# skit-ai/N-Best-ASR-Transformer

Hardware: AMD Instinct MI355X
Metric: utterances/sec fine-tune (bert-base, seq128, n_best=5) (higher is better)
Workload: dtype bf16

## Files before the change

### n-best-asr-transformer_amd/csrc/attention.hip

```cpp
#include "common.h"

namespace {

__device__ __forceinline__ int crow(int reg, int hh) { return (reg & 3) + 8 * (reg >> 2) + 4 * hh; }
__device__ __forceinline__ int gsw(int row) { return ((row >> 2) & 3) | (((row >> 1) & 1) << 2); }

__global__ __launch_bounds__(128) void attn_fwd_f32_kernel(const float* __restrict__ qkv, const uint8_t* __restrict__ mask,
                                                           float* __restrict__ ctx, float* __restrict__ lse, int S, int heads,
                                                           int H, float scale, DropCfg drop) {
  const int bh = blockIdx.x, b = bh / heads, h = bh - b * heads;
  const int i = blockIdx.y * blockDim.x + threadIdx.x;
  if (i >= S) return;
  const int64_t ld = 3 * (int64_t)H;
  const float* base = qkv + (int64_t)b * S * ld;
  const float* qp = base + i * ld + h * 64;
  float q[64];
#pragma unroll
  for (int d = 0; d < 64; ++d) q[d] = qp[d];
  float mx = -INFINITY, l = 0.f;
  for (int j = 0; j < S; ++j) {
    if (!mask[b * S + j]) continue;
    const float* kp = base + j * ld + H + h * 64;
    float s = 0.f;
#pragma unroll
// ... 232 lines not shown
  for (int qb = wave; qb < (kOne ? wave + 1 : NKB); qb += 4) {
    const int q0 = 32 * qb, qrow = q0 + (lane & 31);
    const bool active = qb < NKB;
    if (!kOne) load_q(qb, qf);
    f32x16 sc[NKB];
    if (active) {
#pragma unroll
    for (int kb = 0; kb < NKB; ++kb) {
      f32x16 a;
#pragma unroll
      for (int r = 0; r < 16; ++r) a[r] = 0.f;
#pragma unroll
      for (int ks = 0; ks < 4; ++ks) a = __builtin_amdgcn_mfma_f32_32x32x16_bf16(row_frag(Kt, 32 * kb, ks, lane), qf[ks], a, 0, 0, 0);
      sc[kb] = a;
    }
    }
    if (kOne) __syncthreads();
    if (!active) continue;
    float mx = -INFINITY;
#pragma unroll
    for (int kb = 0; kb < NKB; ++kb)
#pragma unroll
      for (int r4 = 0; r4 < 4; ++r4) {
        const f32x4 ma = *(const f32x4*)(madd + 32 * kb + 8 * r4 + 4 * hh);
#pragma unroll
        for (int e = 0; e < 4; ++e) {
          const float v = sc[kb][4 * r4 + e] * sl2 + ma[e];
          sc[kb][4 * r4 + e] = v;
          mx = fmaxf(mx, v);
        }
      }
    mx = fmaxf(mx, __shfl_xor(mx, 32, 64));
    const float mxs = (mx == -INFINITY) ? 0.f : mx;
    float sum = 0.f;
#pragma unroll
    for (int kb = 0; kb < NKB; ++kb)
#pragma unroll
      for (int r = 0; r < 16; ++r) {
        const float pv = __builtin_amdgcn_exp2f(sc[kb][r] - mxs);
        sc[kb][r] = pv;
        sum += pv;
      }
    sum += __shfl_xor(sum, 32, 64);
    const float inv = 1.0f / sum;
    if (hh == 0 && qrow < S) lse[(int64_t)bh * S + qrow] = mxs * 0.6931471805599453f + __logf(sum);
    bf16x8 pa[NKB][2];
    if (DROP && drop.thr16 && (S & 1) == 0) {
      const uint32_t rowbase = (uint32_t)((bh * S + qrow) * S);
      const uint32_t hb = ((rowbase >> 1) + 2u * (uint32_t)hh) * 0x9E3779B9U + drop.key;
      const float ids = inv * drop.scale;
#pragma unroll
      for (int kb = 0; kb < NKB; ++kb) {
        uint32_t kw = 0;
#pragma unroll
        for (int r = 0; r < 16; r += 2) {
          const uint32_t hsh = nb_hash32(hb + (uint32_t)((32 * kb + crow(r, 0)) >> 1) * 0x9E3779B9U);
          const bool k0 = (hsh & 0xFFFFu) >= drop.thr16, k1 = (hsh >> 16) >= drop.thr16;
          const float p0 = k0 ? sc[kb][r] * ids : 0.f;
          const float p1 = k1 ? sc[kb][r + 1] * ids : 0.f;
          kw |= (k0 ? (1u << crow(r, 0)) : 0u) | (k1 ? (2u << crow(r, 0)) : 0u);
          pa[kb][r >> 3][r & 7] = (bf16)p0;
          pa[kb][r >> 3][(r & 7) + 1] = (bf16)p1;
        }
        if (keep_out) {
          kw <<= 4 * hh;
          kw |= (uint32_t)__shfl_xor((int)kw, 32, 64);
          if (hh == 0 && qrow < Sp) keep_out[((int64_t)bh * NKB + kb) * Sp + qrow] = kw;
        }
      }
    } else {
#pragma unroll
      for (int kb = 0; kb < NKB; ++kb) {
        uint32_t kw = 0;
#pragma unroll
        for (int r = 0; r < 16; ++r) {
          float pv = sc[kb][r] * inv;
          if (DROP && drop.thr16) {
            const int key = 32 * kb + crow(r, hh);
            const bool kp = nb_keep(drop, (uint32_t)((bh * S + qrow) * S + key));
            pv = kp ? pv * drop.scale : 0.f;
            kw |= kp ? (1u << crow(r, hh)) : 0u;
          }
          pa[kb][r >> 3][r & 7] = (bf16)pv;
        }
        if (DROP && keep_out && drop.thr16) {
          kw |= (uint32_t)__shfl_xor((int)kw, 32, 64);
          if (hh == 0 && qrow < Sp) keep_out[((int64_t)bh * NKB + kb) * Sp + qrow] = kw;
        }
      }
    }
    f32x16 o0, o1;
#pragma unroll
    for (int r = 0; r < 16; ++r) o0[r] = o1[r] = 0.f;
#pragma unroll
    for (int kb = 0; kb < NKB; ++kb)
#pragma unroll
      for (int s = 0; s < 2; ++s) {
        o0 = __builtin_amdgcn_mfma_f32_32x32x16_bf16(pa[kb][s], tr_frag<true>(Vt, 32 * kb + 16 * s, 0, lane), o0, 0, 0, 0);
        o1 = __builtin_amdgcn_mfma_f32_32x32x16_bf16(pa[kb][s], tr_frag<true>(Vt, 32 * kb + 16 * s, 32, lane), o1, 0, 0, 0);
      }
    store_tile(Ost + wave * 4096, 0, o0, o1, lane, ctx + ((int64_t)b * S + q0) * H + h * 64, H, S - q0,
               ctx8 ? ctx8 + ((int64_t)b * S + q0) * H + h * 64 : nullptr, s8, amax8, a_new != nullptr);
  }
  if (a_new) {
    amax8 = wave_max(amax8);
    if (lane == 0) amax_update(a_new, amax8);
  }
}

template <int NKB, bool KB>
__global__ __launch_bounds__((NKB <= 4 ? 4 : 8) * 64, 2) void attn_bwd2_bf16_kernel(
    const bf16* __restrict__ qkv, const uint8_t* __restrict__ mask, const bf16* __restrict__ ctx, const bf16* __restrict__ dctx,
    const float* __restrict__ lse, bf16* __restrict__ dqkv, float* __restrict__ colpart, int S, int heads, int H, float scale,
    DropCfg drop, Fp8Grad f8, const uint32_t* __restrict__ keep) {
  extern __shared__ __attribute__((aligned(16))) char lds[];
  constexpr int Sp = NKB * 32;
  constexpr int NW = (NKB <= 4) ? 4 : 8, NT = NW * 64;
  char* Qt = lds;
  char* Kt = Qt + Sp * 128;
  char* dOt = Kt + Sp * 128;
  char* dST = dOt + Sp * 128;
  float* lse_s = (float*)(dST + Sp * 128);
  float* del_s = lse_s + Sp;
  uint32_t* kw_s = (uint32_t*)(del_s + Sp);
  const int tid = threadIdx.x, lane = tid & 63, wave = tid >> 6, hh = lane >> 5;
  const int bh = blockIdx.x, b = bh / heads, h = bh - b * heads;
  const int ld = 3 * H;
  const bf16* base = qkv + (int64_t)b * S * ld;
  const bf16* dobase = dctx + (int64_t)b * S * H;
  const bf16* obase = ctx + (int64_t)b * S * H;
  const __amdgpu_buffer_rsrc_t rs = __builtin_amdgcn_make_buffer_rsrc((void*)base, 0, (uint32_t)(S * ld * 2), 0x00020000);
  const __amdgpu_buffer_rsrc_t rsd = __builtin_amdgcn_make_buffer_rsrc((void*)dobase, 0, (uint32_t)(S * H * 2), 0x00020000);
  stage_rows(rs, Qt, Sp, h * 64, ld, tid, NT);
  stage_rows(rs, Kt, Sp, H + h * 64, ld, tid, NT);
  stage_rows(rsd, dOt, Sp, h * 64, H, tid, NT);
  for (int k = tid; k < Sp; k += NT) lse_s[k] = (k < S) ? lse[(int64_t)bh * S + k] * 1.4426950408889634f : INFINITY;
  if (KB) {
    for (int i = tid; i < NKB * Sp; i += NT) kw_s[i] = keep[(int64_t)bh * NKB * Sp + i];
  }
  {
    const int r = tid >> 1, half = tid & 1;
    float sdel = 0.f;
    if (r < S) {
      const bf16* dp = dobase + (int64_t)r * H + h * 64 + 32 * half;
      const bf16* op = obase + (int64_t)r * H + h * 64 + 32 * half;
#pragma unroll
      for (int c = 0; c < 4; ++c) {
        float a[8], o[8];
        Vec8<bf16>::load(dp + 8 * c, a);
        Vec8<bf16>::load(op + 8 * c, o);
#pragma unroll
        for (int j = 0; j < 8; ++j) sdel = fmaf(a[j], o[j], sdel);
      }
    }
    sdel += __shfl_xor(sdel, 1, 64);
    if (half == 0 && r < Sp) del_s[r] = sdel;
  }
  const int key = 32 * wave + (lane & 31);
  const bool kvalid = (wave < NKB) && key < S;
  const float mk = (kvalid && mask[b * S + key]) ? 0.f : -INFINITY;
  const uint32_t lanebit = 1u << (lane & 31);
  const float sl2 = scale * 1.4426950408889634f;
  bf16x8 kf[4], vf[4];
#pragma unroll
  for (int ks = 0; ks < 4; ++ks) {
    const i32x4 raw = kvalid ? *(const i32x4*)(base + (int64_t)key * ld + 2 * H + h * 64 + 16 * ks + 8 * hh) : i32x4{0, 0, 0, 0};
    vf[ks] = __builtin_bit_cast(bf16x8, raw);
  }
  asm volatile("s_waitcnt vmcnt(0)" ::: "memory");
  __syncthreads();
  if (wave < NKB) {
#pragma unroll
    for (int ks = 0; ks < 4; ++ks) kf[ks] = row_frag(Kt, 32 * wave, ks, lane);
  }
  f32x16 dk0, dk1, dv0, dv1, dq0, dq1;
#pragma unroll
  for (int r = 0; r < 16; ++r) dk0[r] = dk1[r] = dv0[r] = dv1[r] = dq0[r] = dq1[r] = 0.f;
  char* dsrow = dST + key * 128;
  const int dsg = gsw(key);

#pragma unroll 1
  for (int qb = 0; qb < NKB; ++qb) {
    const int half = qb & 1;
    if (wave < NKB) {
      f32x16 sa, da;
#pragma unroll
      for (int r = 0; r < 16; ++r) sa[r] = da[r] = 0.f;
#pragma unroll
      for (int ks = 0; ks < 4; ++ks) {
        sa = __builtin_amdgcn_mfma_f32_32x32x16_bf16(row_frag(Qt, 32 * qb, ks, lane), kf[ks], sa, 0, 0, 0);
        da = __builtin_amdgcn_mfma_f32_32x32x16_bf16(row_frag(dOt, 32 * qb, ks, lane), vf[ks], da, 0, 0, 0);
      }
#pragma unroll
      for (int r4 = 0; r4 < 4; ++r4) {
        const int qoff = 32 * qb + 8 * r4 + 4 * hh;
        const f32x4 l4 = *(const f32x4*)(lse_s + qoff);
        const f32x4 d4 = *(const f32x4*)(del_s + qoff);
        i32x4 k4 = {0, 0, 0, 0};
        if (KB) k4 = *(const i32x4*)(kw_s + wave * Sp + qoff);
        bf16x4 pk;
#pragma unroll
        for (int e = 0; e < 4; ++e) {
          const int r = 4 * r4 + e;
          const float pv = __builtin_amdgcn_exp2f(fmaf(sa[r], sl2, mk - l4[e]));
          float pt = pv, dp = da[r];
          if (KB) {
            const float kf_ = ((uint32_t)k4[e] & lanebit) ? drop.scale : 0.f;
            pt = pv * kf_;
            dp = dp * kf_;
          } else if (drop.thr16) {
            const bool keep_ = nb_keep(drop, (uint32_t)((bh * S + qoff + e) * S + key));
            pt = keep_ ? pv * drop.scale : 0.f;
            dp = keep_ ? dp * drop.scale : 0.f;
          }
          const float ds = pv * (dp - d4[e]) * scale;
          sa[r] = pt;
          da[r] = ds;
          pk[e] = (bf16)ds;
        }
        const int col = 32 * half + 8 * r4 + 4 * hh;
        *(bf16x4*)(dsrow + (((col >> 3) ^ dsg) << 4) + ((col & 4) ? 8 : 0)) = pk;
      }
#pragma unroll
      for (int s2 = 0; s2 < 2; ++s2) {
        const bf16x8 pa = acc_to_frag(sa, s2), dsa = acc_to_frag(da, s2);
        dv0 = __builtin_amdgcn_mfma_f32_32x32x16_bf16(pa, tr_frag<true>(dOt, 32 * qb + 16 * s2, 0, lane), dv0, 0, 0, 0);
        dv1 = __builtin_amdgcn_mfma_f32_32x32x16_bf16(pa, tr_frag<true>(dOt, 32 * qb + 16 * s2, 32, lane), dv1, 0, 0, 0);
        dk0 = __builtin_amdgcn_mfma_f32_32x32x16_bf16(dsa, tr_frag<true>(Qt, 32 * qb + 16 * s2, 0, lane), dk0, 0, 0, 0);
        dk1 = __builtin_amdgcn_mfma_f32_32x32x16_bf16(dsa, tr_frag<true>(Qt, 32 * qb + 16 * s2, 32, lane), dk1, 0, 0, 0);
      }
    }
    __syncthreads();
    if (wave == (qb % NW)) {
#pragma unroll
      for (int ks = 0; ks < 2 * NKB; ++ks) {
        const bf16x8 dsf = tr_frag<false>(dST, 16 * ks, 32 * half, lane);
        dq0 = __builtin_amdgcn_mfma_f32_32x32x16_bf16(dsf, tr_frag<false>(Kt, 16 * ks, 0, lane), dq0, 0, 0, 0);
        dq1 = __builtin_amdgcn_mfma_f32_32x32x16_bf16(dsf, tr_frag<false>(Kt, 16 * ks, 32, lane), dq1, 0, 0, 0);
      }
    }
  }
  __syncthreads();
  if (colpart) {
    float* cs = (float*)dST;
    const f32x16* tiles[6] = {&dq0, &dq1, &dk0, &dk1, &dv0, &dv1};
#pragma unroll
    for (int t6 = 0; t6 < 6; ++t6) {
      float x = 0.f;
      if (wave < NKB) {
#pragma unroll
        for (int r = 0; r < 16; ++r) x += (*tiles[t6])[r];
      }
      x += __shfl_xor(x, 32, 64);
      if (lane < 32) cs[(wave * 3 + (t6 >> 1)) * 64 + (t6 & 1) * 32 + lane] = x;
    }
    __syncthreads();
    if (tid < 192) {
      const int which = tid >> 6, dcol = tid & 63;
      float x = 0.f;
#pragma unroll
      for (int w2 = 0; w2 < NW; ++w2) x += cs[(w2 * 3 + which) * 64 + dcol];
      colpart[(int64_t)b * 3 * H + which * H + h * 64 + dcol] = x;
    }
  }
  if (wave < NKB) {
    const int r0 = 32 * wave;
    const int64_t goff = ((int64_t)b * S + r0) * ld + h * 64;
    bf16* g = dqkv ? dqkv + goff : nullptr;
    uint8_t* g8 = f8.out8 ? f8.out8 + goff : nullptr;
    const float s8 = fp8_grad_scale(f8.amax_prev);
    float amax8 = 0.f;
    const bool am = f8.amax_new != nullptr;
    store_tile(Qt, r0, dq0, dq1, lane, g, ld, S - r0, g8, s8, amax8, am);
    store_tile(Kt, r0, dk0, dk1, lane, g ? g + H : nullptr, ld, S - r0, g8 ? g8 + H : nullptr, s8, amax8, am);
    store_tile(dOt, r0, dv0, dv1, lane, g ? g + 2 * H : nullptr, ld, S - r0, g8 ? g8 + 2 * H : nullptr, s8, amax8, am);
    if (f8.amax_new) {
      amax8 = wave_max(amax8);
      if (lane == 0) amax_update(f8.amax_new, amax8);
    }
  }
}


__device__ __forceinline__ bf16x8 row_frag16(const char* tile, int row0, int ks, int lane) {
  const int row = row0 + (lane & 15);
  const int c = 4 * ks + (lane >> 4);
  return *(const bf16x8*)(tile + row * 128 + ((c ^ gsw(row)) << 4));
}
template <bool PERMUTED>
__device__ __forceinline__ bf16x8 tr_frag16(const char* tile, int kbase, int col0, int lane) {
  const int g = lane >> 4, i = lane & 15, qq = i >> 2, pq = i & 3;
  const int col = col0 + 4 * pq;
  const int r1 = kbase + (PERMUTED ? 4 * g : 8 * g) + qq;
  const int r2 = r1 + (PERMUTED ? 16 : 4);
  const char* a1 = tile + r1 * 128 + (((col >> 3) ^ gsw(r1)) << 4) + ((col & 4) ? 8 : 0);
  const char* a2 = tile + r2 * 128 + (((col >> 3) ^ gsw(r2)) << 4) + ((col & 4) ? 8 : 0);
  const bf16x4 v1 = __builtin_amdgcn_ds_read_tr16_b64_v4bf16((bf16x4 __attribute__((address_space(3)))*)a1);
  const bf16x4 v2 = __builtin_amdgcn_ds_read_tr16_b64_v4bf16((bf16x4 __attribute__((address_space(3)))*)a2);
  bf16x8 o;
  o[0] = v1[0]; o[1] = v1[1]; o[2] = v1[2]; o[3] = v1[3]; o[4] = v2[0]; o[5] = v2[1]; o[6] = v2[2]; o[7] = v2[3];
  return o;
}

template <int NKB, bool KB>
__global__ __launch_bounds__(NKB * 128, 4) void attn_bwd3_bf16_kernel(
    const bf16* __restrict__ qkv, const uint8_t* __restrict__ mask, const bf16* __restrict__ ctx, const bf16* __restrict__ dctx,
    const float* __restrict__ lse, bf16* __restrict__ dqkv, float* __restrict__ colpart, int S, int heads, int H, float scale,
    DropCfg drop, Fp8Grad f8, const uint32_t* __restrict__ keep) {
  extern __shared__ __attribute__((aligned(16))) char lds[];
  static_assert(NKB == 4 || NKB == 8, "attn_bwd3: 8 or 16 waves of 16 keys");
  constexpr int Sp = NKB * 32, NW = 2 * NKB, NT = NW * 64;
  char* Qt = lds;
  char* Kt = Qt + Sp * 128;
  char* dOt = Kt + Sp * 128;
  char* dST = dOt + Sp * 128;
  float* lse_s = (float*)(dST + Sp * 128);
  float* del_s = lse_s + Sp;
  uint32_t* kw_s = (uint32_t*)(del_s + Sp);
  const int tid = threadIdx.x, lane = tid & 63, wave = tid >> 6, g = lane >> 4, c16 = lane & 15;
  const int bh = blockIdx.x, b = bh / heads, h = bh - b * heads;
  const int ld = 3 * H;
  const bf16* base = qkv + (int64_t)b * S * ld;
  const bf16* dobase = dctx + (int64_t)b * S * H;
  const bf16* obase = ctx + (int64_t)b * S * H;
  const __amdgpu_buffer_rsrc_t rs = __builtin_amdgcn_make_buffer_rsrc((void*)base, 0, (uint32_t)(S * ld * 2), 0x00020000);
  const __amdgpu_buffer_rsrc_t rsd = __builtin_amdgcn_make_buffer_rsrc((void*)dobase, 0, (uint32_t)(S * H * 2), 0x00020000);
  stage_rows(rs, Qt, Sp, h * 64, ld, tid, NT);
  stage_rows(rs, Kt, Sp, H + h * 64, ld, tid, NT);
  stage_rows(rsd, dOt, Sp, h * 64, H, tid, NT);
  for (int k = tid; k < Sp; k += NT) lse_s[k] = (k < S) ? lse[(int64_t)bh * S + k] * 1.4426950408889634f : INFINITY;
  if (KB) {
    for (int i = tid; i < NKB * Sp; i += NT) kw_s[i] = keep[(int64_t)bh * NKB * Sp + i];
  }
  {
    const int r = tid >> 2, quarter = tid & 3;
    float sdel = 0.f;
    if (r < S) {
      const bf16* dp = dobase + (int64_t)r * H + h * 64 + 16 * quarter;
      const bf16* op = obase + (int64_t)r * H + h * 64 + 16 * quarter;
#pragma unroll
      for (int c = 0; c < 2; ++c) {
        float a[8], o[8];
        Vec8<bf16>::load(dp + 8 * c, a);
        Vec8<bf16>::load(op + 8 * c, o);
#pragma unroll
        for (int j = 0; j < 8; ++j) sdel = fmaf(a[j], o[j], sdel);
      }
    }
    sdel += __shfl_xor(sdel, 1, 64);
    sdel += __shfl_xor(sdel, 2, 64);
    if (quarter == 0 && r < Sp) del_s[r] = sdel;
  }
  const int key = 16 * wave + c16;
  const bool kvalid = key < S;
  const float mk = (kvalid && mask[b * S + key]) ? 0.f : -INFINITY;
  const uint32_t lanebit = 1u << (key & 31);
  const float sl2 = scale * 1.4426950408889634f;
  bf16x8 kf[2], vf[2];
#pragma unroll
  for (int ks = 0; ks < 2; ++ks) {
    const i32x4 raw = kvalid ? *(const i32x4*)(base + (int64_t)key * ld + 2 * H + h * 64 + 32 * ks + 8 * g) : i32x4{0, 0, 0, 0};
    vf[ks] = __builtin_bit_cast(bf16x8, raw);
  }
  asm volatile("s_waitcnt vmcnt(0)" ::: "memory");
  __syncthreads();
#pragma unroll
  for (int ks = 0; ks < 2; ++ks) kf[ks] = row_frag16(Kt, 16 * wave, ks, lane);
  f32x4 dk[4], dv[4], dq[4];
#pragma unroll
  for (int t = 0; t < 4; ++t) { dk[t] = f32x4{0, 0, 0, 0}; dv[t] = f32x4{0, 0, 0, 0}; }
#pragma unroll
  for (int t = 0; t < 4; ++t) dq[t] = f32x4{0, 0, 0, 0};
  char* dsrow = dST + key * 128;
  const int dsg = gsw(key);
  const int qt_mine = (wave & 7) >> 2, dt_mine = wave & 3;
  const int khalf = wave >> 3;

#pragma unroll
  for (int qb = 0; qb < NKB; ++qb) {
    const int half = qb & 1;
    f32x4 sa[2], da[2];
#pragma unroll
    for (int qt = 0; qt < 2; ++qt) {
      sa[qt] = f32x4{0, 0, 0, 0}; da[qt] = f32x4{0, 0, 0, 0};
#pragma unroll
      for (int ks = 0; ks < 2; ++ks) {
        sa[qt] = __builtin_amdgcn_mfma_f32_16x16x32_bf16(row_frag16(Qt, 32 * qb + 16 * qt, ks, lane), kf[ks], sa[qt], 0, 0, 0);
        da[qt] = __builtin_amdgcn_mfma_f32_16x16x32_bf16(row_frag16(dOt, 32 * qb + 16 * qt, ks, lane), vf[ks], da[qt], 0, 0, 0);
      }
    }
    bf16x8 pa, dsa;
#pragma unroll
    for (int qt = 0; qt < 2; ++qt) {
      const int qoff = 32 * qb + 16 * qt + 4 * g;
      const f32x4 l4 = *(const f32x4*)(lse_s + qoff);
      const f32x4 d4 = *(const f32x4*)(del_s + qoff);
      i32x4 k4 = {0, 0, 0, 0};
      if (KB) k4 = *(const i32x4*)(kw_s + (wave >> 1) * Sp + qoff);
      bf16x4 pk;
#pragma unroll
      for (int e = 0; e < 4; ++e) {
        const float pv = __builtin_amdgcn_exp2f(fmaf(sa[qt][e], sl2, mk - l4[e]));
        float pt = pv, dp = da[qt][e];
        if (KB) {
          const float kf_ = ((uint32_t)k4[e] & lanebit) ? drop.scale : 0.f;
          pt = pv * kf_;
          dp = dp * kf_;
        } else if (drop.thr16) {
          const bool keep_ = nb_keep(drop, (uint32_t)((bh * S + qoff + e) * S + key));
          pt = keep_ ? pv * drop.scale : 0.f;
          dp = keep_ ? dp * drop.scale : 0.f;
        }
        const float ds = pv * (dp - d4[e]) * scale;
        pa[4 * qt + e] = (bf16)pt;
        dsa[4 * qt + e] = (bf16)ds;
        pk[e] = (bf16)ds;
      }
      const int col = 32 * half + 16 * qt + 4 * g;
      *(bf16x4*)(dsrow + (((col >> 3) ^ dsg) << 4) + ((col & 4) ? 8 : 0)) = pk;
    }
#pragma unroll
    for (int dt = 0; dt < 4; ++dt) {
      dv[dt] = __builtin_amdgcn_mfma_f32_16x16x32_bf16(pa, tr_frag16<true>(dOt, 32 * qb, 16 * dt, lane), dv[dt], 0, 0, 0);
      dk[dt] = __builtin_amdgcn_mfma_f32_16x16x32_bf16(dsa, tr_frag16<true>(Qt, 32 * qb, 16 * dt, lane), dk[dt], 0, 0, 0);
    }
    __syncthreads();
    if (NKB == 4 || (qb & 1) == khalf) {
      const int slot = (NKB == 4) ? qb : (qb >> 1);
#pragma unroll
      for (int ks = 0; ks < NKB; ++ks)
        dq[slot] = __builtin_amdgcn_mfma_f32_16x16x32_bf16(tr_frag16<false>(dST, 32 * ks, 32 * half + 16 * qt_mine, lane),
                                                           tr_frag16<false>(Kt, 32 * ks, 16 * dt_mine, lane), dq[slot], 0, 0, 0);
    }
  }
  __syncthreads();
  if (colpart) {
    float* cs = (float*)dST;
    float* csq = cs + NW * 2 * 64;
#pragma unroll
    for (int dt = 0; dt < 4; ++dt) {
      float xk = (dk[dt][0] + dk[dt][1]) + (dk[dt][2] + dk[dt][3]);
      float xv = (dv[dt][0] + dv[dt][1]) + (dv[dt][2] + dv[dt][3]);
      xk += __shfl_xor(xk, 16, 64); xk += __shfl_xor(xk, 32, 64);
      xv += __shfl_xor(xv, 16, 64); xv += __shfl_xor(xv, 32, 64);
      if (g == 0) { cs[(wave * 2 + 0) * 64 + 16 * dt + c16] = xk; cs[(wave * 2 + 1) * 64 + 16 * dt + c16] = xv; }
    }
    float xq = 0.f;
#pragma unroll
    for (int t = 0; t < 4; ++t) xq += (dq[t][0] + dq[t][1]) + (dq[t][2] + dq[t][3]);
    xq += __shfl_xor(xq, 16, 64); xq += __shfl_xor(xq, 32, 64);
    if (g == 0) csq[wave * 16 + c16] = xq;
    __syncthreads();
    if (tid < 192) {
      const int which = tid >> 6, dcol = tid & 63;
      float x = 0.f;
      if (which == 0) {
#pragma unroll
        for (int w2 = 0; w2 < NW / 4; ++w2) x += csq[((dcol >> 4) + 4 * w2) * 16 + (dcol & 15)];
      }
      else {
#pragma unroll
        for (int w2 = 0; w2 < NW; ++w2) x += cs[(w2 * 2 + (which - 1)) * 64 + dcol];
      }
      colpart[(int64_t)b * 3 * H + which * H + h * 64 + dcol] = x;
    }
    __syncthreads();
  }
#pragma unroll
  for (int dt = 0; dt < 4; ++dt)
#pragma unroll
    for (int e = 0; e < 4; ++e) {
      const int row = 16 * wave + 4 * g + e;
      *(bf16*)(Kt + row * 128 + (16 * dt + c16) * 2) = (bf16)dk[dt][e];
      *(bf16*)(dOt + row * 128 + (16 * dt + c16) * 2) = (bf16)dv[dt][e];
    }
#pragma unroll
  for (int t = 0; t < 4; ++t) {
    const int qb = (NKB == 4) ? t : 2 * t + khalf;
#pragma unroll
    for (int e = 0; e < 4; ++e)
      *(bf16*)(Qt + (32 * qb + 16 * qt_mine + 4 * g + e) * 128 + (16 * dt_mine + c16) * 2) = (bf16)dq[t][e];
  }
  __syncthreads();
  {
    const int64_t goff = (int64_t)b * S * ld + h * 64;
    bf16* gq = dqkv ? dqkv + goff : nullptr;
    uint8_t* g8 = f8.out8 ? f8.out8 + goff : nullptr;
    const float s8 = fp8_grad_scale(f8.amax_prev);
    const bool am = f8.amax_new != nullptr;
    float amax8 = 0.f;
    const char* imgs[3] = {Qt, Kt, dOt};
#pragma unroll
    for (int t = 0; t < 3; ++t) {
#pragma unroll
      for (int it = 0; it < (Sp * 8) / NT; ++it) {
        const int p = it * NT + tid, row = p >> 3, ch = p & 7;
        if (row < S) {
          const i32x4 v = *(const i32x4*)(imgs[t] + row * 128 + ch * 16);
          if (gq) *(i32x4*)(gq + (int64_t)row * ld + t * H + ch * 8) = v;
          if (g8 || am) {
            const bf16x8 bb = __builtin_bit_cast(bf16x8, v);
            float f[8];
#pragma unroll
            for (int e = 0; e < 8; ++e) f[e] = (float)bb[e];
            if (am) {
#pragma unroll
              for (int e = 0; e < 8; ++e) amax8 = fmaxf(amax8, fabsf(f[e]));
            }
            if (g8) {
#pragma unroll
              for (int e = 0; e < 8; ++e) f[e] *= s8;
              *(i32x2*)(g8 + (int64_t)row * ld + t * H + ch * 8) = i32x2{(int)fp8_pack4(f), (int)fp8_pack4(f + 4)};
            }
          }
        }
      }
    }
    if (am) {
      amax8 = wave_max(amax8);
      if (lane == 0) amax_update(f8.amax_new, amax8);
    }
  }
}


__device__ __forceinline__ void stage_rows_off(__amdgpu_buffer_rsrc_t rs, char* tile, int nrows, int row_off, int col_off, int ld,
                                               int t, int nt) {
  const int chunks = nrows * 8;
  for (int p = t; p < chunks; p += nt) {
    const int row = p >> 3, slot = p & 7;
    const int c = slot ^ gsw(row);
    const uint32_t voff = (uint32_t)(((row_off + row) * ld + col_off + c * 8) * 2);
    __builtin_amdgcn_raw_ptr_buffer_load_lds(rs, LDS_PTR(tile + (p & ~63) * 16), 16, voff, 0, 0, 0);
  }
}

__global__ __launch_bounds__(256) void attn_fwd_long_bf16_kernel(const bf16* __restrict__ qkv, const uint8_t* __restrict__ mask,
                                                                 bf16* __restrict__ ctx, float* __restrict__ lse, int S, int nkb,
                                                                 int heads, int H, float scale, DropCfg drop, uint8_t* __restrict__ ctx8,
                                                                 const uint32_t* __restrict__ a_prev, uint32_t* __restrict__ a_new) {
  const float s8 = fp8_act_scale(a_prev);
  float amax8 = 0.f;
  extern __shared__ __attribute__((aligned(16))) char lds[];
  const int Sp = nkb * 32;
  char* Kt = lds;
  char* Vt = lds + Sp * 128;
  float* madd = (float*)(lds + 2 * Sp * 128);
  char* Ost = lds + 2 * Sp * 128 + Sp * 4;
  const int tid = threadIdx.x, lane = tid & 63, wave = tid >> 6, hh = lane >> 5;
  const int bh = blockIdx.x, b = bh / heads, h = bh - b * heads;
  const int ld = 3 * H;
  const bf16* base = qkv + (int64_t)b * S * ld;
  const __amdgpu_buffer_rsrc_t rs = __builtin_amdgcn_make_buffer_rsrc((void*)base, 0, (uint32_t)(S * ld * 2), 0x00020000);
  stage_rows(rs, Kt, Sp, H + h * 64, ld, tid);
  stage_rows(rs, Vt, Sp, 2 * H + h * 64, ld, tid);
  for (int k = tid; k < Sp; k += 256) madd[k] = (k < S && mask[b * S + k]) ? 0.f : -INFINITY;
  asm volatile("s_waitcnt vmcnt(0)" ::: "memory");
  __syncthreads();

  for (int qb = wave; qb < nkb; qb += 4) {
    const int q0 = 32 * qb, qrow = q0 + (lane & 31);
    bf16x8 qf[4];
#pragma unroll
    for (int ks = 0; ks < 4; ++ks) {
      const i32x4 raw = (qrow < S) ? *(const i32x4*)(base + (int64_t)qrow * ld + h * 64 + 16 * ks + 8 * hh) : i32x4{0, 0, 0, 0};
      qf[ks] = __builtin_bit_cast(bf16x8, raw);
    }
    float m = -INFINITY, l = 0.f;
#pragma unroll 1
    for (int kb = 0; kb < nkb; ++kb) {
      f32x16 a;
#pragma unroll
      for (int r = 0; r < 16; ++r) a[r] = 0.f;
#pragma unroll
      for (int ks = 0; ks < 4; ++ks) a = __builtin_amdgcn_mfma_f32_32x32x16_bf16(row_frag(Kt, 32 * kb, ks, lane), qf[ks], a, 0, 0, 0);
      float bm = -INFINITY;
#pragma unroll
      for (int r4 = 0; r4 < 4; ++r4) {
        const f32x4 ma = *(const f32x4*)(madd + 32 * kb + 8 * r4 + 4 * hh);
#pragma unroll
        for (int e = 0; e < 4; ++e) {
          const float v = a[4 * r4 + e] * scale + ma[e];
          a[4 * r4 + e] = v;
          bm = fmaxf(bm, v);
        }
      }
      const float mn = fmaxf(m, bm);
      if (mn > -INFINITY) {
        float add = 0.f;
#pragma unroll
        for (int r = 0; r < 16; ++r) add += __expf(a[r] - mn);
        l = ((m > -INFINITY) ? l * __expf(m - mn) : 0.f) + add;
      }
      m = mn;
    }
    const float mo = __shfl_xor(m, 32, 64), lo = __shfl_xor(l, 32, 64);
    const float mx = fmaxf(m, mo);
    const float mxs = (mx == -INFINITY) ? 0.f : mx;
    const float sum = ((m > -INFINITY) ? l * __expf(m - mxs) : 0.f) + ((mo > -INFINITY) ? lo * __expf(mo - mxs) : 0.f);
    const float inv = 1.0f / sum;
    if (hh == 0 && qrow < S) lse[(int64_t)bh * S + qrow] = mxs + __logf(sum);
    f32x16 o0, o1;
#pragma unroll
    for (int r = 0; r < 16; ++r) o0[r] = o1[r] = 0.f;
    const uint32_t rowbase = (uint32_t)((bh * S + qrow) * S);
    const bool pair_hash = drop.thr16 && (S & 1) == 0;
#pragma unroll 1
    for (int kb = 0; kb < nkb; ++kb) {
      f32x16 a;
#pragma unroll
      for (int r = 0; r < 16; ++r) a[r] = 0.f;
#pragma unroll
      for (int ks = 0; ks < 4; ++ks) a = __builtin_amdgcn_mfma_f32_32x32x16_bf16(row_frag(Kt, 32 * kb, ks, lane), qf[ks], a, 0, 0, 0);
#pragma unroll
      for (int r4 = 0; r4 < 4; ++r4) {
        const f32x4 ma = *(const f32x4*)(madd + 32 * kb + 8 * r4 + 4 * hh);
#pragma unroll
        for (int e = 0; e < 4; ++e) a[4 * r4 + e] = __expf(a[4 * r4 + e] * scale + ma[e] - mxs) * inv;
      }
      if (pair_hash) {
#pragma unroll
        for (int r = 0; r < 16; r += 2) {
          const uint32_t idx = rowbase + (uint32_t)(32 * kb + crow(r, hh));
          const uint32_t hsh = nb_hash32((idx >> 1) * 0x9E3779B9U + drop.key);
          a[r] = ((hsh & 0xFFFFu) >= drop.thr16) ? a[r] * drop.scale : 0.f;
          a[r + 1] = ((hsh >> 16) >= drop.thr16) ? a[r + 1] * drop.scale : 0.f;
        }
      } else if (drop.thr16) {
#pragma unroll
        for (int r = 0; r < 16; ++r) a[r] = nb_keep(drop, rowbase + (uint32_t)(32 * kb + crow(r, hh))) ? a[r] * drop.scale : 0.f;
      }
#pragma unroll
      for (int s = 0; s < 2; ++s) {
        const bf16x8 pa = acc_to_frag(a, s);
        o0 = __builtin_amdgcn_mfma_f32_32x32x16_bf16(pa, tr_frag<true>(Vt, 32 * kb + 16 * s, 0, lane), o0, 0, 0, 0);
        o1 = __builtin_amdgcn_mfma_f32_32x32x16_bf16(pa, tr_frag<true>(Vt, 32 * kb + 16 * s, 32, lane), o1, 0, 0, 0);
      }
    }
    store_tile(Ost + wave * 4096, 0, o0, o1, lane, ctx + ((int64_t)b * S + q0) * H + h * 64, H, S - q0,
               ctx8 ? ctx8 + ((int64_t)b * S + q0) * H + h * 64 : nullptr, s8, amax8, a_new != nullptr);
  }
  if (a_new) {
    amax8 = wave_max(amax8);
    if (lane == 0) amax_update(a_new, amax8);
  }
}

__global__ __launch_bounds__(512) void attn_bwd_long_bf16_kernel(const bf16* __restrict__ qkv, const uint8_t* __restrict__ mask,
                                                                 const bf16* __restrict__ ctx, const bf16* __restrict__ dctx,
                                                                 const float* __restrict__ lse, bf16* __restrict__ dqkv,
                                                                 float* __restrict__ colpart, int S, int nkb, int heads, int H,
                                                                 float scale, DropCfg drop, Fp8Grad f8) {
  extern __shared__ __attribute__((aligned(16))) char lds[];
  constexpr int NW = 8, NT = 512, KH = 256, RS = 512;
  const float s8 = fp8_grad_scale(f8.amax_prev);
  float amax8 = 0.f;
  const bool am = f8.amax_new != nullptr;
  const int Sp = nkb * 32;
  char* Qs = lds;
  char* dOs = Qs + 2 * 4096;
  char* Kt = dOs + 2 * 4096;
  char* dSb = Kt + KH * 128;
  float* lse_s = (float*)(dSb + 2 * 32 * RS);
  float* del_s = lse_s + Sp;
  const int tid = threadIdx.x, lane = tid & 63, wave = tid >> 6, hh = lane >> 5;
  const int bh = blockIdx.x, b = bh / heads, h = bh - b * heads;
  const int ld = 3 * H;
  const bf16* base = qkv + (int64_t)b * S * ld;
  const bf16* dobase = dctx + (int64_t)b * S * H;
  const bf16* obase = ctx + (int64_t)b * S * H;
  const __amdgpu_buffer_rsrc_t rs = __builtin_amdgcn_make_buffer_rsrc((void*)base, 0, (uint32_t)(S * ld * 2), 0x00020000);
  const __amdgpu_buffer_rsrc_t rsd = __builtin_amdgcn_make_buffer_rsrc((void*)dobase, 0, (uint32_t)(S * H * 2), 0x00020000);
  for (int k = tid; k < Sp; k += NT) lse_s[k] = (k < S) ? lse[(int64_t)bh * S + k] : INFINITY;
  for (int r = tid >> 1; r < Sp; r += NT / 2) {
    const int half = tid & 1;
    float sdel = 0.f;
    if (r < S) {
      const bf16* dp = dobase + (int64_t)r * H + h * 64 + 32 * half;
      const bf16* op = obase + (int64_t)r * H + h * 64 + 32 * half;
#pragma unroll
      for (int c = 0; c < 4; ++c) {
        float a[8], o[8];
        Vec8<bf16>::load(dp + 8 * c, a);
        Vec8<bf16>::load(op + 8 * c, o);
#pragma unroll
        for (int j = 0; j < 8; ++j) sdel = fmaf(a[j], o[j], sdel);
      }
    }
    sdel += __shfl_xor(sdel, 1, 64);
    if (half == 0) del_s[r] = sdel;
  }
  f32x16 dqa0, dqa1, dqb0, dqb1;
  float ck0 = 0.f, ck1 = 0.f, cv0 = 0.f, cv1 = 0.f;
#pragma unroll
  for (int r = 0; r < 16; ++r) dqa0[r] = dqa1[r] = dqb0[r] = dqb1[r] = 0.f;
  const int nkh = (nkb + 7) / 8;

#pragma unroll 1
  for (int kh = 0; kh < nkh; ++kh) {
    const int key0 = KH * kh;
    const int nkb_h = (nkb - 8 * kh < 8) ? nkb - 8 * kh : 8;
    __syncthreads();
    stage_rows_off(rs, Kt, KH, key0, H + h * 64, ld, tid, NT);
    if (wave < 4) stage_rows_off(rs, Qs, 32, 0, h * 64, ld, tid, 256);
    else stage_rows_off(rsd, dOs, 32, 0, h * 64, H, tid - 256, 256);
    const int keyl = 32 * wave + (lane & 31), key = key0 + keyl;
    const bool active = wave < nkb_h;
    const bool kvalid = active && key < S;
    const float mk = (kvalid && mask[b * S + key]) ? 0.f : -INFINITY;
    const bf16* vrow = base + (int64_t)(kvalid ? key : 0) * ld + 2 * H + h * 64 + 8 * hh;
    asm volatile("s_waitcnt vmcnt(0)" ::: "memory");
    __syncthreads();
    f32x16 dk0, dk1, dv0, dv1;
#pragma unroll
    for (int r = 0; r < 16; ++r) dk0[r] = dk1[r] = dv0[r] = dv1[r] = 0.f;

#pragma unroll 1
    for (int qb = 0; qb < nkb; ++qb) {
      const int cur = qb & 1;
      const char* Qc = Qs + cur * 4096;
      const char* dOc = dOs + cur * 4096;
      char* slab = dSb + cur * 32 * RS;
      if (qb + 1 < nkb) {
        if (wave < 4) stage_rows_off(rs, Qs + (cur ^ 1) * 4096, 32, 32 * (qb + 1), h * 64, ld, tid, 256);
        else stage_rows_off(rsd, dOs + (cur ^ 1) * 4096, 32, 32 * (qb + 1), h * 64, H, tid - 256, 256);
      }
      if (active) {
        f32x16 sa, da;
#pragma unroll
        for (int r = 0; r < 16; ++r) sa[r] = da[r] = 0.f;
#pragma unroll
        for (int ks = 0; ks < 4; ++ks) {
          const i32x4 raw = kvalid ? *(const i32x4*)(vrow + 16 * ks) : i32x4{0, 0, 0, 0};
          sa = __builtin_amdgcn_mfma_f32_32x32x16_bf16(row_frag(Qc, 0, ks, lane), row_frag(Kt, 32 * wave, ks, lane), sa, 0, 0, 0);
          da = __builtin_amdgcn_mfma_f32_32x32x16_bf16(row_frag(dOc, 0, ks, lane), __builtin_bit_cast(bf16x8, raw), da, 0, 0, 0);
        }
#pragma unroll
        for (int r4 = 0; r4 < 4; ++r4) {
          const f32x4 l4 = *(const f32x4*)(lse_s + 32 * qb + 8 * r4 + 4 * hh);
          const f32x4 d4 = *(const f32x4*)(del_s + 32 * qb + 8 * r4 + 4 * hh);
#pragma unroll
          for (int e = 0; e < 4; ++e) {
            const int r = 4 * r4 + e;
            const int ql = 8 * r4 + 4 * hh + e;
            const int q = 32 * qb + ql;
            const float pv = __expf(sa[r] * scale + mk - l4[e]);
            float pt = pv, dp = da[r];
            if (drop.thr16) {
              const bool keep = nb_keep(drop, (uint32_t)((bh * S + q) * S + key));
              pt = keep ? pv * drop.scale : 0.f;
              dp = keep ? dp * drop.scale : 0.f;
            }
            const float ds = pv * (dp - d4[e]) * scale;
            sa[r] = pt;
            da[r] = ds;
            *(bf16*)(slab + ql * RS + ((((keyl >> 3) ^ (ql & 15))) << 4) + (keyl & 7) * 2) = (bf16)ds;
          }
        }
#pragma unroll
        for (int s2 = 0; s2 < 2; ++s2) {
          const bf16x8 pa = acc_to_frag(sa, s2), dsa = acc_to_frag(da, s2);
          dv0 = __builtin_amdgcn_mfma_f32_32x32x16_bf16(pa, tr_frag<true>(dOc, 16 * s2, 0, lane), dv0, 0, 0, 0);
          dv1 = __builtin_amdgcn_mfma_f32_32x32x16_bf16(pa, tr_frag<true>(dOc, 16 * s2, 32, lane), dv1, 0, 0, 0);
          dk0 = __builtin_amdgcn_mfma_f32_32x32x16_bf16(dsa, tr_frag<true>(Qc, 16 * s2, 0, lane), dk0, 0, 0, 0);
          dk1 = __builtin_amdgcn_mfma_f32_32x32x16_bf16(dsa, tr_frag<true>(Qc, 16 * s2, 32, lane), dk1, 0, 0, 0);
        }
      }
      asm volatile("s_waitcnt vmcnt(0)" ::: "memory");
      __syncthreads();
      if (wave == (qb & 7)) {
#define NB_DQ_ACC(D0, D1)                                                                                      \
  _Pragma("unroll 1") for (int ks = 0; ks < 2 * nkb_h; ++ks) {                                                 \
    const int row = lane & 31;                                                                                 \
    const int c = 2 * ks + hh;                                                                                 \
    const bf16x8 dsf = *(const bf16x8*)(slab + row * RS + ((c ^ (row & 15)) << 4));                            \
    D0 = __builtin_amdgcn_mfma_f32_32x32x16_bf16(dsf, tr_frag<false>(Kt, 16 * ks, 0, lane), D0, 0, 0, 0);      \
    D1 = __builtin_amdgcn_mfma_f32_32x32x16_bf16(dsf, tr_frag<false>(Kt, 16 * ks, 32, lane), D1, 0, 0, 0);     \
  }
        if (qb < 8) { NB_DQ_ACC(dqa0, dqa1) } else { NB_DQ_ACC(dqb0, dqb1) }
#undef NB_DQ_ACC
      }
    }
    __syncthreads();
    if (active) {
#pragma unroll
      for (int r = 0; r < 16; ++r) { ck0 += dk0[r]; ck1 += dk1[r]; cv0 += dv0[r]; cv1 += dv1[r]; }
      const int r0 = key0 + 32 * wave;
      const int64_t goff = ((int64_t)b * S + r0) * ld + h * 64;
      bf16* g = dqkv ? dqkv + goff : nullptr;
      uint8_t* g8 = f8.out8 ? f8.out8 + goff : nullptr;
      store_tile(Kt + wave * 4096, 0, dk0, dk1, lane, g ? g + H : nullptr, ld, S - r0, g8 ? g8 + H : nullptr, s8, amax8, am);
      store_tile(Kt + wave * 4096, 0, dv0, dv1, lane, g ? g + 2 * H : nullptr, ld, S - r0, g8 ? g8 + 2 * H : nullptr, s8, amax8, am);
    }
  }
  __syncthreads();
  if (colpart) {
    float* cs = (float*)dSb;
    float cq0 = 0.f, cq1 = 0.f;
#pragma unroll
    for (int r = 0; r < 16; ++r) { cq0 += dqa0[r] + dqb0[r]; cq1 += dqa1[r] + dqb1[r]; }
    float v6[6] = {cq0, cq1, ck0, ck1, cv0, cv1};
#pragma unroll
    for (int t6 = 0; t6 < 6; ++t6) {
      float x = v6[t6];
      x += __shfl_xor(x, 32, 64);
      if (lane < 32) cs[(wave * 3 + (t6 >> 1)) * 64 + (t6 & 1) * 32 + lane] = x;
    }
    __syncthreads();
    if (tid < 192) {
      const int which = tid >> 6, dcol = tid & 63;
      float x = 0.f;
#pragma unroll
      for (int w2 = 0; w2 < NW; ++w2) x += cs[(w2 * 3 + which) * 64 + dcol];
      colpart[(int64_t)b * 3 * H + which * H + h * 64 + dcol] = x;
    }
  }
  if (wave < nkb) {
    const int r0 = 32 * wave;
    const int64_t goff = ((int64_t)b * S + r0) * ld + h * 64;
    store_tile(Kt + wave * 4096, 0, dqa0, dqa1, lane, dqkv ? dqkv + goff : nullptr, ld, S - r0, f8.out8 ? f8.out8 + goff : nullptr, s8, amax8, am);
  }
  if (wave + 8 < nkb) {
    const int r0 = 32 * (wave + 8);
    const int64_t goff = ((int64_t)b * S + r0) * ld + h * 64;
// ... 640 lines not shown
```

Measured before the change: 13110.

## Pipeline attention backward dQ stores and staging with per-block waits

Specializes the single-block attention backward kernel to 8 waves (S ≤ 128). It stages Q and dO per 32-row block through buffer loads into LDS and waits on them block by block with explicit vmcnt counts. Each dQ block is computed into one accumulator and written out during the next iteration, so global stores overlap with compute instead of all happening at the end. The upfront global loads (mask, lse, delta inputs, V, keep bits) switch to buffer intrinsics with fewer barriers, and the NKB=8 path is dropped. The hand-counted waitcnts are fragile: a miscount would read LDS before it is filled.

```diff
diff --git a/n-best-asr-transformer_amd/csrc/attention.hip b/n-best-asr-transformer_amd/csrc/attention.hip
--- a/n-best-asr-transformer_amd/csrc/attention.hip
+++ b/n-best-asr-transformer_amd/csrc/attention.hip
@@ -558,13 +558,43 @@
   return o;
 }
 
+__device__ __forceinline__ void bwd3_store_chunk(const char* img, int row, int ch, __amdgpu_buffer_rsrc_t rq, bool gq,
+                                                 __amdgpu_buffer_rsrc_t r8, bool g8, int ld, int col0, float s8, bool am, float& amax8) {
+  const u32x4 v = *(const u32x4*)(img + row * 128 + ch * 16);
+  const int eoff = row * ld + col0 + ch * 8;
+  if (gq) __builtin_amdgcn_raw_buffer_store_b128(v, rq, eoff * 2, 0, 0);
+  if (g8 || am) {
+    const bf16x8 bb = __builtin_bit_cast(bf16x8, v);
+    float f[8];
+#pragma unroll
+    for (int e = 0; e < 8; ++e) f[e] = (float)bb[e];
+    if (am) {
+#pragma unroll
+      for (int e = 0; e < 8; ++e) amax8 = fmaxf(amax8, fabsf(f[e]));
+    }
+    if (g8) {
+#pragma unroll
+      for (int e = 0; e < 8; ++e) f[e] *= s8;
+      __builtin_amdgcn_raw_buffer_store_b64(u32x2{fp8_pack4(f), fp8_pack4(f + 4)}, r8, eoff, 0, 0);
+    }
+  }
+}
+
+#define BWD3_PIN() asm volatile("" ::: "memory")
+#define BWD3_VMCNT(n) asm volatile("s_waitcnt vmcnt(" #n ")" ::: "memory")
+__device__ __forceinline__ void bwd3_barrier() {
+  asm volatile("s_waitcnt lgkmcnt(0)" ::: "memory");
+  __builtin_amdgcn_s_barrier();
+  BWD3_PIN();
+}
+
 template <int NKB, bool KB>
 __global__ __launch_bounds__(NKB * 128, 4) void attn_bwd3_bf16_kernel(
     const bf16* __restrict__ qkv, const uint8_t* __restrict__ mask, const bf16* __restrict__ ctx, const bf16* __restrict__ dctx,
     const float* __restrict__ lse, bf16* __restrict__ dqkv, float* __restrict__ colpart, int S, int heads, int H, float scale,
     DropCfg drop, Fp8Grad f8, const uint32_t* __restrict__ keep) {
   extern __shared__ __attribute__((aligned(16))) char lds[];
-  static_assert(NKB == 4 || NKB == 8, "attn_bwd3: 8 or 16 waves of 16 keys");
+  static_assert(NKB == 4, "attn_bwd3: 8 waves of 16 keys, 96 < S <= 128");
   constexpr int Sp = NKB * 32, NW = 2 * NKB, NT = NW * 64;
   char* Qt = lds;
   char* Kt = Qt + Sp * 128;
@@ -581,56 +611,83 @@
   const bf16* obase = ctx + (int64_t)b * S * H;
   const __amdgpu_buffer_rsrc_t rs = __builtin_amdgcn_make_buffer_rsrc((void*)base, 0, (uint32_t)(S * ld * 2), 0x00020000);
   const __amdgpu_buffer_rsrc_t rsd = __builtin_amdgcn_make_buffer_rsrc((void*)dobase, 0, (uint32_t)(S * H * 2), 0x00020000);
-  stage_rows(rs, Qt, Sp, h * 64, ld, tid, NT);
+  const int wv = __builtin_amdgcn_readfirstlane(wave);
+  constexpr int kOut = 0x40000000;
+  const __amdgpu_buffer_rsrc_t rso = __builtin_amdgcn_make_buffer_rsrc((void*)obase, 0, (uint32_t)(S * H * 2), 0x00020000);
+  const bool isq = wv < 4;
+  const __amdgpu_buffer_rsrc_t rsb = __builtin_amdgcn_make_buffer_rsrc((void*)(isq ? base : dobase), 0,
+                                                                       (uint32_t)(S * (isq ? ld : H) * 2), 0x00020000);
+  auto stage_block = [&](int qb) {
+    const int row0 = 32 * qb + 8 * (wv & 3), row = row0 + (lane >> 3);
+    const int c = (lane & 7) ^ gsw(row);
+    const uint32_t voff = (uint32_t)((row * (isq ? ld : H) + h * 64 + c * 8) * 2);
+    __builtin_amdgcn_raw_ptr_buffer_load_lds(rsb, LDS_PTR((isq ? Qt : dOt) + row0 * 128), 16, voff, 0, 0, 0);
+    BWD3_PIN();
+  };
   stage_rows(rs, Kt, Sp, H + h * 64, ld, tid, NT);
-  stage_rows(rsd, dOt, Sp, h * 64, H, tid, NT);
-  for (int k = tid; k < Sp; k += NT) lse_s[k] = (k < S) ? lse[(int64_t)bh * S + k] * 1.4426950408889634f : INFINITY;
-  if (KB) {
-    for (int i = tid; i < NKB * Sp; i += NT) kw_s[i] = keep[(int64_t)bh * NKB * Sp + i];
-  }
-  {
-    const int r = tid >> 2, quarter = tid & 3;
-    float sdel = 0.f;
-    if (r < S) {
-      const bf16* dp = dobase + (int64_t)r * H + h * 64 + 16 * quarter;
-      const bf16* op = obase + (int64_t)r * H + h * 64 + 16 * quarter;
-#pragma unroll
-      for (int c = 0; c < 2; ++c) {
-        float a[8], o[8];
-        Vec8<bf16>::load(dp + 8 * c, a);
-        Vec8<bf16>::load(op + 8 * c, o);
-#pragma unroll
-        for (int j = 0; j < 8; ++j) sdel = fmaf(a[j], o[j], sdel);
-      }
-    }
-    sdel += __shfl_xor(sdel, 1, 64);
-    sdel += __shfl_xor(sdel, 2, 64);
-    if (quarter == 0 && r < Sp) del_s[r] = sdel;
-  }
+  BWD3_PIN();
   const int key = 16 * wave + c16;
-  const bool kvalid = key < S;
-  const float mk = (kvalid && mask[b * S + key]) ? 0.f : -INFINITY;
+  const __amdgpu_buffer_rsrc_t rsm = __builtin_amdgcn_make_buffer_rsrc((void*)(mask + (int64_t)b * S), 0, (uint32_t)S, 0x00020000);
+  const __amdgpu_buffer_rsrc_t rsl = __builtin_amdgcn_make_buffer_rsrc((void*)(lse + (int64_t)bh * S), 0, (uint32_t)(S * 4), 0x00020000);
+  const __amdgpu_buffer_rsrc_t rsa = __builtin_amdgcn_make_buffer_rsrc((void*)f8.amax_prev, 0, f8.amax_prev ? 4u : 0u, 0x00020000);
+  const uint8_t mbyte = __builtin_amdgcn_raw_buffer_load_b8(rsm, key, 0, 0);
   const uint32_t lanebit = 1u << (key & 31);
   const float sl2 = scale * 1.4426950408889634f;
   bf16x8 kf[2], vf[2];
 #pragma unroll
-  for (int ks = 0; ks < 2; ++ks) {
-    const i32x4 raw = kvalid ? *(const i32x4*)(base + (int64_t)key * ld + 2 * H + h * 64 + 32 * ks + 8 * g) : i32x4{0, 0, 0, 0};
-    vf[ks] = __builtin_bit_cast(bf16x8, raw);
-  }
-  asm volatile("s_waitcnt vmcnt(0)" ::: "memory");
-  __syncthreads();
+  for (int ks = 0; ks < 2; ++ks)
+    vf[ks] = __builtin_bit_cast(bf16x8, __builtin_amdgcn_raw_buffer_load_b128(rs, (key * ld + 2 * H + h * 64 + 32 * ks + 8 * g) * 2, 0, 0));
+  const uint32_t lse_raw = __builtin_amdgcn_raw_buffer_load_b32(rsl, tid < Sp ? tid * 4 : kOut, 0, 0);
+  const uint32_t amax_raw = __builtin_amdgcn_raw_buffer_load_b32(rsa, 0, 0, 0);
+  uint32_t kw_k = 0;
+  if (KB) kw_k = keep[(int64_t)bh * NKB * Sp + tid];
+  {
+    const int r = tid >> 2, quarter = tid & 3;
+    bf16x8 a[2], o[2];
+#pragma unroll
+    for (int c = 0; c < 2; ++c) {
+      const int voff = (r * H + h * 64 + 16 * quarter + 8 * c) * 2;
+      a[c] = __builtin_bit_cast(bf16x8, __builtin_amdgcn_raw_buffer_load_b128(rsd, voff, 0, 0));
+      o[c] = __builtin_bit_cast(bf16x8, __builtin_amdgcn_raw_buffer_load_b128(rso, voff, 0, 0));
+    }
+    BWD3_PIN();
+#pragma unroll
+    for (int qb = 0; qb < NKB; ++qb) stage_block(qb);
+    float* lse_dst = (tid < Sp) ? lse_s + tid : (float*)dST + tid;
+    *lse_dst = (tid < S) ? __uint_as_float(lse_raw) * 1.4426950408889634f : INFINITY;
+    if (KB) kw_s[tid] = kw_k;
+    float sdel = 0.f;
+#pragma unroll
+    for (int c = 0; c < 2; ++c)
+#pragma unroll
+      for (int j = 0; j < 8; ++j) sdel = fmaf((float)a[c][j], (float)o[c][j], sdel);
+    sdel = dpp_add<0xB1>(sdel);
+    sdel = dpp_add<0x4E>(sdel);
+    if (quarter == 0) del_s[r] = sdel;
+  }
+  const float mk = mbyte ? 0.f : -INFINITY;
+  BWD3_VMCNT(3);
+  bwd3_barrier();
 #pragma unroll
   for (int ks = 0; ks < 2; ++ks) kf[ks] = row_frag16(Kt, 16 * wave, ks, lane);
-  f32x4 dk[4], dv[4], dq[4];
+  f32x4 dk[4], dv[4];
 #pragma unroll
   for (int t = 0; t < 4; ++t) { dk[t] = f32x4{0, 0, 0, 0}; dv[t] = f32x4{0, 0, 0, 0}; }
-#pragma unroll
-  for (int t = 0; t < 4; ++t) dq[t] = f32x4{0, 0, 0, 0};
+  float xq = 0.f;
   char* dsrow = dST + key * 128;
   const int dsg = gsw(key);
-  const int qt_mine = (wave & 7) >> 2, dt_mine = wave & 3;
-  const int khalf = wave >> 3;
+  const int qt_mine = wave >> 2, dt_mine = wave & 3;
+  const int64_t goff = (int64_t)b * S * ld + h * 64;
+  const bool gq = dqkv != nullptr, g8 = f8.out8 != nullptr;
+  const __amdgpu_buffer_rsrc_t rq = __builtin_amdgcn_make_buffer_rsrc((void*)(gq ? dqkv + goff : nullptr), 0, gq ? (uint32_t)((S * ld - h * 64) * 2) : 0u, 0x00020000);
+  const __amdgpu_buffer_rsrc_t r8 = __builtin_amdgcn_make_buffer_rsrc((void*)(g8 ? f8.out8 + goff : nullptr), 0, g8 ? (uint32_t)(S * ld - h * 64) : 0u, 0x00020000);
+  const float s8 = f8.amax_prev ? fp8_gscale_of(__uint_as_float(__builtin_amdgcn_readfirstlane(amax_raw))) : 1.f;
+  const bool am = f8.amax_new != nullptr;
+  float amax8 = 0.f;
+  auto store_dq_block = [&](int qb) {
+    const int p = 32 * wave + lane, row = 32 * qb + (p >> 3);
+    if (lane < 32 && row < S) bwd3_store_chunk(Qt, row, p & 7, rq, gq, r8, g8, ld, 0, s8, am, amax8);
+  };
 
 #pragma unroll
   for (int qb = 0; qb < NKB; ++qb) {
@@ -680,14 +737,24 @@
       dv[dt] = __builtin_amdgcn_mfma_f32_16x16x32_bf16(pa, tr_frag16<true>(dOt, 32 * qb, 16 * dt, lane), dv[dt], 0, 0, 0);
       dk[dt] = __builtin_amdgcn_mfma_f32_16x16x32_bf16(dsa, tr_frag16<true>(Qt, 32 * qb, 16 * dt, lane), dk[dt], 0, 0, 0);
     }
-    __syncthreads();
-    if (NKB == 4 || (qb & 1) == khalf) {
-      const int slot = (NKB == 4) ? qb : (qb >> 1);
-#pragma unroll
-      for (int ks = 0; ks < NKB; ++ks)
-        dq[slot] = __builtin_amdgcn_mfma_f32_16x16x32_bf16(tr_frag16<false>(dST, 32 * ks, 32 * half + 16 * qt_mine, lane),
-                                                           tr_frag16<false>(Kt, 32 * ks, 16 * dt_mine, lane), dq[slot], 0, 0, 0);
-    }
+    if (qb == 0) BWD3_VMCNT(2);
+    if (qb == 1) BWD3_VMCNT(1);
+    if (qb == 2) {
+      if (gq && g8) BWD3_VMCNT(2);
+      else if (gq || g8) BWD3_VMCNT(1);
+      else BWD3_VMCNT(0);
+    }
+    bwd3_barrier();
+    if (qb >= 1) store_dq_block(qb - 1);
+    f32x4 dq = {0, 0, 0, 0};
+#pragma unroll
+    for (int ks = 0; ks < NKB; ++ks)
+      dq = __builtin_amdgcn_mfma_f32_16x16x32_bf16(tr_frag16<false>(dST, 32 * ks, 32 * half + 16 * qt_mine, lane),
+                                                   tr_frag16<false>(Kt, 32 * ks, 16 * dt_mine, lane), dq, 0, 0, 0);
+    xq += (dq[0] + dq[1]) + (dq[2] + dq[3]);
+#pragma unroll
+    for (int e = 0; e < 4; ++e)
+      *(bf16*)(Qt + (32 * qb + 16 * qt_mine + 4 * g + e) * 128 + (16 * dt_mine + c16) * 2) = (bf16)dq[e];
   }
   __syncthreads();
   if (colpart) {
@@ -701,9 +768,6 @@
       xv += __shfl_xor(xv, 16, 64); xv += __shfl_xor(xv, 32, 64);
       if (g == 0) { cs[(wave * 2 + 0) * 64 + 16 * dt + c16] = xk; cs[(wave * 2 + 1) * 64 + 16 * dt + c16] = xv; }
     }
-    float xq = 0.f;
-#pragma unroll
-    for (int t = 0; t < 4; ++t) xq += (dq[t][0] + dq[t][1]) + (dq[t][2] + dq[t][3]);
     xq += __shfl_xor(xq, 16, 64); xq += __shfl_xor(xq, 32, 64);
     if (g == 0) csq[wave * 16 + c16] = xq;
     __syncthreads();
@@ -722,60 +786,29 @@
     }
     __syncthreads();
   }
+  const int lane_e = __builtin_amdgcn_mbcnt_hi(~0u, __builtin_amdgcn_mbcnt_lo(~0u, 0u));
 #pragma unroll
   for (int dt = 0; dt < 4; ++dt)
 #pragma unroll
     for (int e = 0; e < 4; ++e) {
-      const int row = 16 * wave + 4 * g + e;
-      *(bf16*)(Kt + row * 128 + (16 * dt + c16) * 2) = (bf16)dk[dt][e];
-      *(bf16*)(dOt + row * 128 + (16 * dt + c16) * 2) = (bf16)dv[dt][e];
-    }
-#pragma unroll
-  for (int t = 0; t < 4; ++t) {
-    const int qb = (NKB == 4) ? t : 2 * t + khalf;
-#pragma unroll
-    for (int e = 0; e < 4; ++e)
-      *(bf16*)(Qt + (32 * qb + 16 * qt_mine + 4 * g + e) * 128 + (16 * dt_mine + c16) * 2) = (bf16)dq[t][e];
-  }
+      const int row = 16 * wv + 4 * (lane_e >> 4) + e;
+      *(bf16*)(Kt + row * 128 + (16 * dt + (lane_e & 15)) * 2) = (bf16)dk[dt][e];
+      *(bf16*)(dOt + row * 128 + (16 * dt + (lane_e & 15)) * 2) = (bf16)dv[dt][e];
+    }
   __syncthreads();
-  {
-    const int64_t goff = (int64_t)b * S * ld + h * 64;
-    bf16* gq = dqkv ? dqkv + goff : nullptr;
-    uint8_t* g8 = f8.out8 ? f8.out8 + goff : nullptr;
-    const float s8 = fp8_grad_scale(f8.amax_prev);
-    const bool am = f8.amax_new != nullptr;
-    float amax8 = 0.f;
-    const char* imgs[3] = {Qt, Kt, dOt};
-#pragma unroll
-    for (int t = 0; t < 3; ++t) {
-#pragma unroll
-      for (int it = 0; it < (Sp * 8) / NT; ++it) {
-        const int p = it * NT + tid, row = p >> 3, ch = p & 7;
-        if (row < S) {
-          const i32x4 v = *(const i32x4*)(imgs[t] + row * 128 + ch * 16);
-          if (gq) *(i32x4*)(gq + (int64_t)row * ld + t * H + ch * 8) = v;
-          if (g8 || am) {
-            const bf16x8 bb = __builtin_bit_cast(bf16x8, v);
-            float f[8];
-#pragma unroll
-            for (int e = 0; e < 8; ++e) f[e] = (float)bb[e];
-            if (am) {
-#pragma unroll
-              for (int e = 0; e < 8; ++e) amax8 = fmaxf(amax8, fabsf(f[e]));
-            }
-            if (g8) {
-#pragma unroll
-              for (int e = 0; e < 8; ++e) f[e] *= s8;
-              *(i32x2*)(g8 + (int64_t)row * ld + t * H + ch * 8) = i32x2{(int)fp8_pack4(f), (int)fp8_pack4(f + 4)};
-            }
-          }
-        }
-      }
-    }
-    if (am) {
-      amax8 = wave_max(amax8);
-      if (lane == 0) amax_update(f8.amax_new, amax8);
-    }
+  store_dq_block(NKB - 1);
+  const char* imgs[2] = {Kt, dOt};
+#pragma unroll
+  for (int t = 0; t < 2; ++t) {
+#pragma unroll
+    for (int it = 0; it < (Sp * 8) / NT; ++it) {
+      const int p = it * NT + tid, row = p >> 3;
+      if (row < S) bwd3_store_chunk(imgs[t], row, p & 7, rq, gq, r8, g8, ld, (t + 1) * H, s8, am, amax8);
+    }
+  }
+  if (am) {
+    amax8 = wave_max(amax8);
+    if (lane == 0) amax_update(f8.amax_new, amax8);
   }
 }
 
```

Result: no change. 13160, median of 6 (+0.4%).
